# mchitten/keto

Measured on AMD Instinct MI355X. Metric: permission checks/sec (batched, whole node) + traversal HBM GB/s vs roofline, higher is better.
Workload: dtype u32 ids / u64 bitmasks (integer)

## Files before the change

include/ketogpu.h:

```cpp
#ifndef KETOGPU_H
#define KETOGPU_H

#include <stddef.h>
#include <stdint.h>

#ifdef __cplusplus
extern "C" {
#endif

#define KETOGPU_ABI_VERSION 9

#define KETOGPU_OK 0
#define KETOGPU_ENOTFOUND 1
#define KETOGPU_EINVAL 2
#define KETOGPU_EDEVICE 3
#define KETOGPU_ENOMEM 4
#define KETOGPU_ECOLLISION 5

#define KETOGPU_SUBJECT_ID 0
#define KETOGPU_SUBJECT_SET 1
#define KETOGPU_SUBJECT_NIL (-1)

#define KETOGPU_NODE_NONE 0xFFFFFFFFu
#define KETOGPU_NODE_NOT_OWNED 0xFFFFFFFEu
// ... 187 lines not shown
                      uint64_t *allowed_bits, uint64_t *flagged_bits);

size_t ketogpu_packed24_bytes(size_t n);
int ketogpu_pack24(const uint32_t *roots, const uint32_t *targets, size_t n, void *out);
int ketogpu_unpack24(const void *packed, size_t n, uint32_t *roots, uint32_t *targets);
int ketogpu_snapshot_packed24_ok(const ketogpu_snapshot *s);
int ketogpu_check_ids_packed24(ketogpu_engine *e, const void *packed, size_t n, uint64_t *allowed_bits,
                               uint64_t *flagged_bits);
int ketogpu_engine_last_request_path(const ketogpu_engine *e, int32_t *path);

int ketogpu_host_alloc(size_t bytes, void **out);
void ketogpu_host_free(void *p);

typedef struct ketogpu_multi ketogpu_multi;
int ketogpu_multi_new(const ketogpu_snapshot *s, const int32_t *devices, size_t num_devices,
                      const ketogpu_engine_opts *opts, ketogpu_multi **out);
void ketogpu_multi_free(ketogpu_multi *m);
size_t ketogpu_multi_size(const ketogpu_multi *m);
ketogpu_engine *ketogpu_multi_engine(ketogpu_multi *m, size_t i);
int ketogpu_multi_check_ids(ketogpu_multi *m, const uint32_t *roots, const uint32_t *targets, size_t n,
                            uint64_t *allowed_bits, uint64_t *flagged_bits);
int ketogpu_multi_check_ids_packed24(ketogpu_multi *m, const void *packed, size_t n, uint64_t *allowed_bits,
                                     uint64_t *flagged_bits);
void ketogpu_multi_range(size_t n, size_t parts, size_t i, size_t *begin, size_t *end);

int ketogpu_queries_upload(ketogpu_engine *e, const uint32_t *roots, const uint32_t *targets,
                           size_t n, ketogpu_queries **out);
int ketogpu_queries_run(ketogpu_engine *e, ketogpu_queries *q);
int ketogpu_queries_download(ketogpu_engine *e, const ketogpu_queries *q, uint64_t *allowed_bits,
                             uint64_t *flagged_bits);
int ketogpu_queries_run_async(ketogpu_engine *e, ketogpu_queries *q, int *queued);
int ketogpu_engine_wait(ketogpu_engine *e);
int ketogpu_engine_piped_full_requests(ketogpu_engine *e, uint64_t *out);
void ketogpu_queries_free(ketogpu_queries *q);

typedef struct {
    uint64_t checks;
    uint64_t rounds;
    uint64_t levels;
    uint64_t frontier_entries;
    uint64_t interior_edges;
    uint64_t rev_edges;
    uint64_t touched;
    uint64_t bytes_push;
    uint64_t bytes_pull;
    uint64_t bytes_total;
    double ms_push;
    double ms_pull;
    double ms_total;
    uint64_t push_launches;
    uint64_t overflow_retries;
    uint64_t spilled_units;
    uint64_t unit_rows;
    uint64_t unit_edges;
    uint64_t unit_rev;
    uint64_t bytes_unit;
    double ms_unit;
    uint64_t spilled_requests;
    uint64_t unit_launches;
    uint64_t main_bytes;
    double main_ms;
    int32_t plan;
    uint32_t plan_lists;
    uint32_t hubs;
    uint32_t hub_words;
    double hub_build_ms;
// ... 502 lines not shown
    uint32_t slots;
    double last_call_ms;
} ketogpu_expand_stats;
int ketogpu_subjects_expand_stats_get(const ketogpu_subjects *h, ketogpu_expand_stats *out);
int ketogpu_subjects_expand(ketogpu_subjects *h, const uint32_t *roots, const uint32_t *rest_depth, size_t n,
                            uint32_t *out_nodes, uint32_t *out_children, uint64_t capacity, uint64_t *begin,
                            uint64_t *count, uint32_t *status, uint64_t *needed);

typedef struct {
    uint64_t requests;
    uint64_t tier1_requests;
    uint64_t wide_requests;
    uint64_t wide_rounds;
    uint64_t levels;
    uint64_t items;
    uint64_t ids_produced;
    uint64_t truncated_lists;
    uint32_t slots;
    uint32_t chunk;
    double last_call_ms;
} ketogpu_wide_stats;
int ketogpu_subjects_wide_stats_get(const ketogpu_subjects *h, ketogpu_wide_stats *out);
int ketogpu_lookup_wide_stats_get(const ketogpu_lookup *l, ketogpu_wide_stats *out);
int ketogpu_subjects_ids_wide(ketogpu_subjects *h, const uint32_t *roots, size_t n, uint32_t cls, uint32_t *out,
                              uint64_t capacity, uint64_t *begin, uint64_t *count, uint64_t *needed);
int ketogpu_lookup_ids_wide(ketogpu_lookup *l, const uint32_t *targets, size_t n, uint32_t type, uint32_t *out,
                            uint64_t capacity, uint64_t *begin, uint64_t *count, uint64_t *needed);

const char *ketogpu_last_error(void);
int ketogpu_abi_version(void);
void ketogpu_free(void *p);
int ketogpu_device_count(void);
int ketogpu_probe_random_lines(int device, uint64_t table_bytes, uint64_t requests, int reps, double *ms_per_launch);

#ifdef __cplusplus
}
#endif
#endif
```

keto_amd/_lib.py:

```python
import ctypes as C
import os

HERE = os.path.dirname(os.path.abspath(__file__))
LIB_PATH = os.environ.get("KETOGPU_LIB") or os.path.join(HERE, "libketogpu.so")

OK, ENOTFOUND, EINVAL, EDEVICE, ENOMEM, ECOLLISION = 0, 1, 2, 3, 4, 5
SUBJECT_ID, SUBJECT_SET, SUBJECT_NIL = 0, 1, -1
NODE_NONE = 0xFFFFFFFF
NODE_NOT_OWNED = 0xFFFFFFFE
BUILD_SORT = 1
ORDER_NULLS_LAST = 2
ORDERS = {"sqlite": 0, "mysql-bin": 0, "cockroach": 0, "postgres": ORDER_NULLS_LAST}
BUILD_WRITABLE = 4
WRITE_REASONS = {0: "applied", 1: "not_writable", 2: "wildcard", 3: "poison", 4: "class", 5: "ambiguous",
                 6: "full", 7: "reserve", 8: "fanout"}
NODE_UNION, NODE_LEAF = 0, 1
TYPE_ANY, TYPE_NONE = 0xFFFFFFFF, 0xFFFFFFFE
LOOKUP_TRUNCATED, LOOKUP_INVALID = 0xFFFFFFFFFFFFFFFF, 0xFFFFFFFFFFFFFFFE
CLASS_SUBJECT_ID, CLASS_UNTYPED_SET = 0xFFFFFFFD, 0xFFFFFFFC
PAGE_LIMIT_MAX, PAGE_INVALID = 65536, 0xFFFFFFFF
COMBINE_AND, COMBINE_ANDNOT, COMBINE_OR = 0, 1, 2


class KetoError(Exception):
# ... 387 lines not shown
    "ketogpu_core_index_free": (None, [vp]),
    "ketogpu_comm_stats_get": (C.c_int, [vp, C.POINTER(CommStats)]),
    "ketogpu_label_index_build": (C.c_int, [vp, u32, u32, C.POINTER(vp)]),
    "ketogpu_label_index_view": (C.c_int, [vp, C.POINTER(LabelView)]),
    "ketogpu_label_index_free": (None, [vp]),
    "ketogpu_engine_label_heads": (C.c_int, [vp, C.c_int, vp, C.c_uint64, C.POINTER(C.c_uint64),
                                             C.POINTER(C.c_uint32)]),
    "ketogpu_snapshot_save": (C.c_int, [vp, C.c_char_p]),
    "ketogpu_snapshot_apply": (C.c_int, [vp, C.POINTER(RowBatch), C.POINTER(RowBatch), C.POINTER(vp)]),
    "ketogpu_snapshot_load": (C.c_int, [C.c_char_p, C.POINTER(vp)]),
    "ketogpu_snapshot_set_namespaces": (C.c_int, [vp, C.POINTER(Namespace), sz, C.POINTER(vp)]),
    "ketogpu_snapshot_write": (C.c_int, [vp, C.POINTER(RowBatch), C.POINTER(RowBatch), C.POINTER(WriteResult)]),
    "ketogpu_snapshot_version": (C.c_uint64, [vp]),
    "ketogpu_engine_sync": (C.c_int, [vp, C.POINTER(C.c_double), C.POINTER(C.c_uint64)]),
    "ketogpu_engine_check_graph": (C.c_int, [vp, C.POINTER(C.c_uint64)]),
    "ketogpu_resolve": (C.c_int, [vp, C.POINTER(CheckRequest), C.POINTER(u32), C.POINTER(u32)]),
    "ketogpu_resolve_batch": (C.c_int, [vp, C.POINTER(RequestBatch), vp, vp, vp]),
    "ketogpu_engine_new": (C.c_int, [vp, C.POINTER(EngineOpts), C.POINTER(vp)]),
    "ketogpu_engine_free": (None, [vp]),
    "ketogpu_engine_set_events": (C.c_int, [vp, C.c_int]),
    "ketogpu_check": (C.c_int, [vp, C.POINTER(CheckRequest), sz, vp, vp]),
    "ketogpu_check_ids": (C.c_int, [vp, vp, vp, sz, vp, vp]),
    "ketogpu_packed24_bytes": (sz, [sz]),
    "ketogpu_pack24": (C.c_int, [vp, vp, sz, vp]),
    "ketogpu_unpack24": (C.c_int, [vp, sz, vp, vp]),
    "ketogpu_snapshot_packed24_ok": (C.c_int, [vp]),
    "ketogpu_check_ids_packed24": (C.c_int, [vp, vp, sz, vp, vp]),
    "ketogpu_engine_last_request_path": (C.c_int, [vp, C.POINTER(i32)]),
    "ketogpu_queries_upload": (C.c_int, [vp, vp, vp, sz, C.POINTER(vp)]),
    "ketogpu_queries_run": (C.c_int, [vp, vp]),
    "ketogpu_queries_run_async": (C.c_int, [vp, vp, C.POINTER(C.c_int)]),
    "ketogpu_engine_wait": (C.c_int, [vp]),
    "ketogpu_engine_piped_full_requests": (C.c_int, [vp, C.POINTER(C.c_uint64)]),
    "ketogpu_probe_random_lines": (C.c_int, [C.c_int, C.c_uint64, C.c_uint64, C.c_int, C.POINTER(C.c_double)]),
    "ketogpu_queries_download": (C.c_int, [vp, vp, vp, vp]),
    "ketogpu_queries_free": (None, [vp]),
    "ketogpu_engine_last_stats": (C.c_int, [vp, C.POINTER(RunStats)]),
    "ketogpu_expand": (C.c_int, [vp, C.POINTER(Subject), i32, C.POINTER(vp)]),
    "ketogpu_tree_nodes": (C.c_int, [vp, C.POINTER(C.POINTER(TreeNode)), C.POINTER(sz)]),
    "ketogpu_tree_json": (C.c_int, [vp, C.POINTER(vp)]),
    "ketogpu_tree_free": (None, [vp]),
    "ketogpu_last_error": (C.c_char_p, []),
    "ketogpu_abi_version": (C.c_int, []),
    "ketogpu_free": (None, [vp]),
    "ketogpu_device_count": (C.c_int, []),
    "ketogpu_host_alloc": (C.c_int, [sz, C.POINTER(vp)]),
    "ketogpu_host_free": (None, [vp]),
    "ketogpu_multi_new": (C.c_int, [vp, vp, sz, C.POINTER(EngineOpts), C.POINTER(vp)]),
    "ketogpu_multi_free": (None, [vp]),
    "ketogpu_multi_size": (sz, [vp]),
    "ketogpu_multi_engine": (vp, [vp, sz]),
    "ketogpu_multi_check_ids": (C.c_int, [vp, vp, vp, sz, vp, vp]),
    "ketogpu_multi_check_ids_packed24": (C.c_int, [vp, vp, sz, vp, vp]),
    "ketogpu_multi_range": (None, [sz, sz, sz, C.POINTER(sz), C.POINTER(sz)]),
    "ketogpu_shard_builder_new": (C.c_int, [C.POINTER(Namespace), sz, C.POINTER(ShardOpts), C.POINTER(vp)]),
    "ketogpu_shard_builder_append": (C.c_int, [vp, C.POINTER(RowBatch)]),
    "ketogpu_shard_builder_finish": (C.c_int, [vp, C.POINTER(vp)]),
    "ketogpu_shard_builder_free": (None, [vp]),
    "ketogpu_shard_free": (None, [vp]),
    "ketogpu_shard_counts": (C.c_int, [vp, vp]),
    "ketogpu_shard_set_layout": (C.c_int, [vp, vp]),
    "ketogpu_shard_query_count": (C.c_uint64, [vp]),
    "ketogpu_shard_queries": (C.c_int, [vp, vp, C.c_uint64, vp]),
    "ketogpu_shard_answer": (C.c_int, [vp, vp, C.c_uint64, vp]),
    "ketogpu_shard_apply": (C.c_int, [vp, vp, C.c_uint64]),
    "ketogpu_shard_claim_count": (C.c_uint64, [vp]),
    "ketogpu_shard_claims": (C.c_int, [vp, vp, C.c_uint64, vp]),
# ... 132 lines not shown
```

keto_amd/check.py:

```python
import ctypes as C

import numpy as np

from . import _lib as L
from .relationtuple import InternalRelationTuple, NilSubject
from .snapshot import Snapshot, subject_struct


class Engine:
    def __init__(self, snapshot: Snapshot, device=0, max_words_per_round=0, state_budget_bytes=0):
        self.L = L.lib()
        self.snapshot = snapshot
        opts = L.EngineOpts(device, max_words_per_round, state_budget_bytes)
        h = C.c_void_p()
        L.check(self.L.ketogpu_engine_new(snapshot.h, C.byref(opts), C.byref(h)))
        self.h = h
        self.owned = True

    @classmethod
    def borrowed(cls, handle, snapshot, owner):
        e = cls.__new__(cls)
        e.L, e.snapshot, e.h, e.owned, e._owner = L.lib(), snapshot, C.c_void_p(handle), False, owner
        return e

# ... 79 lines not shown
        bad = C.c_uint64()
        L.check(self.L.ketogpu_engine_check_graph(self.h, C.byref(bad)))
        self.check_graph_first = self.L.ketogpu_last_error().decode("utf-8", "replace") if bad.value else ""
        return bad.value

    def label_heads(self, side):
        words, hw = C.c_uint64(), C.c_uint32()
        L.check(self.L.ketogpu_engine_label_heads(self.h, side, None, 0, C.byref(words), C.byref(hw)))
        if not words.value:
            return None, 0
        out = np.empty(words.value, dtype=np.uint32)
        L.check(self.L.ketogpu_engine_label_heads(self.h, side, out.ctypes.data, words.value, C.byref(words),
                                                  C.byref(hw)))
        return out, hw.value

    def sync(self):
        ms, rows = C.c_double(), C.c_uint64()
        L.check(self.L.ketogpu_engine_sync(self.h, C.byref(ms), C.byref(rows)))
        return ms.value, rows.value

    def last_stats(self):
        st = L.RunStats()
        L.check(self.L.ketogpu_engine_last_stats(self.h, C.byref(st)))
        return st.as_dict()

    def wait(self):
        L.check(self.L.ketogpu_engine_wait(self.h))

    def piped_full_requests(self):
        n = C.c_uint64()
        L.check(self.L.ketogpu_engine_piped_full_requests(self.h, C.byref(n)))
        return n.value

    def set_events(self, every_kernel):
        L.check(self.L.ketogpu_engine_set_events(self.h, 1 if every_kernel else 0))


class PinnedBuffer:

    def __init__(self, n, dtype=np.uint32):
        self.L = L.lib()
        dt = np.dtype(dtype)
        p = C.c_void_p()
        L.check(self.L.ketogpu_host_alloc(max(n, 1) * dt.itemsize, C.byref(p)))
        self.p = p
        buf = (C.c_char * (max(n, 1) * dt.itemsize)).from_address(p.value)
        self.array = np.frombuffer(buf, dtype=dt)[:n]

    def close(self):
        if getattr(self, "p", None):
            self.array = None
            self.L.ketogpu_host_free(self.p)
            self.p = None

    def __del__(self):
        self.close()


def pinned(values, dtype=np.uint32):
    values = np.asarray(values, dtype=dtype)
    b = PinnedBuffer(len(values), dtype)
    b.array[:] = values
    return b


class MultiEngine:
# ... 143 lines not shown
```

keto_amd/csrc/device_engine.hip:

```cpp
#include <hip/hip_runtime.h>

#include <algorithm>
#include <atomic>
#include <chrono>
#include <cstring>
#include <functional>
#include <map>
#include <mutex>
#include <string>
#include <thread>
#include <type_traits>
#include <vector>

#include "core_index.hpp"
#include "device_util.hpp"
#include "labels.hpp"
#include "tier.hpp"
#include "ketogpu_internal.hpp"

using namespace ketogpu;
using namespace kdev;

namespace {

// ... 2219 lines not shown
template <int E>
__device__ __forceinline__ bool label_find_e(const uint32_t *L, uint32_t x) {
    const uint32_t pos = label_lower_e<E>(L, x);
    return pos < (uint32_t)E && L[pos] == x;
}

template <int E>
__device__ __forceinline__ bool label_block8(const uint32_t *L, uint32_t x) {
    static_assert(E % 8 == 4, "a head's inline entries");
    constexpr int NB = (E + 7) / 8;
    uint32_t blk = 0;
#pragma unroll
    for (int b = 0; b + 1 < NB; b++) blk += L[8 * b + 7] < x;
    const uint4 u = *reinterpret_cast<const uint4 *>(L + 8 * blk);
    const bool lo = min(min(u.x ^ x, u.y ^ x), min(u.z ^ x, u.w ^ x)) == 0;
    if constexpr (NB == 1) {
        return lo;
    } else {
        const uint4 v = *reinterpret_cast<const uint4 *>(L + 8 * blk + 4);
        const bool hi = min(min(v.x ^ x, v.y ^ x), min(v.z ^ x, v.w ^ x)) == 0;
        return lo | (hi & (blk != (uint32_t)(NB - 1)));
    }
}

template <int E, int H>
__device__ __forceinline__ bool label_lookup(const uint32_t *row, uint32_t x) {
    return label_block8<E>(row + kHeadFixed, x);
}

#ifndef KETO_LABEL_MEET
#define KETO_LABEL_MEET 0
#endif

template <int HS, int HP, bool TAIL = false>
__device__ __forceinline__ void label_unit(LabelShared<HS, HP> &sh, const LabelGraph &L, uint32_t r_lane,
                                           uint32_t t_lane, uint64_t *allowed, const uint64_t unit,
                                           const LabelRest &R, const LabelRest &F, unsigned long long *stats) {
    static_assert((HS == 8 || HS == 16 || HS == 32 || HS == 64) && (HP == 8 || HP == 16 || HP == 32 || HP == 64),
                  "heads of 8, 16, 32 or 64 words");
    constexpr int SW = HS / 4, PW = HP / 4;
    constexpr uint32_t CS = HS - kHeadFixed, CP = HP - kHeadFixed;
    const uint32_t lane = threadIdx.x & 63, q = lane >> 2, sub = lane & 3;
    const uint32_t r = (uint32_t)__shfl((int)r_lane, (int)q, 64), t = (uint32_t)__shfl((int)t_lane, (int)q, 64);
    const bool some = r != KETOGPU_NODE_NONE && t != KETOGPU_NODE_NONE;
    const bool valid = some && r < kDynBase;
    uint32_t sw[SW], pw[PW];
#pragma unroll
    for (int k = 0; k < SW; k++) sw[k] = 0xFFFFFFFFu;
#pragma unroll
    for (int k = 0; k < PW; k++) pw[k] = 0xFFFFFFFFu;
    if (valid) {
        label_head_load<SW>(L.S + (uint64_t)t * HS, sub, sw);
        label_head_load<PW>(L.P + (uint64_t)r * HP, sub, pw);
    }
    const uint32_t ns = label_word<SW, 0>(sw), np = label_word<PW, 0>(pw);
    const bool labelled = valid && ns != kNoLabel && np != kNoLabel;
    const uint64_t smask = (uint64_t)label_word<SW, 2>(sw) | (uint64_t)label_word<SW, 3>(sw) << 32;
    const uint64_t pmask = (uint64_t)label_word<PW, 2>(pw) | (uint64_t)label_word<PW, 3>(pw) << 32;
    uint32_t *Sl = sh.S + q * (HS + 4), *Pl = sh.P + q * (HP + 4);
    label_to_lds<SW>(Sl, sw, sub);
    label_to_lds<PW>(Pl, pw, sub);
    const uint32_t *Se = Sl + kHeadFixed, *Pe = Pl + kHeadFixed;
    const uint32_t shard = (uint32_t)(unit % kRestShards);
    {
        const bool rest = sub == 0 && some && !labelled;
        const uint32_t at = lds_append(rest, R.count + shard * kRestStride);
        if (rest) R.list[shard * R.cap + at] = (uint32_t)(unit * 16 + q);
    }
    wave_sync();
    bool hit = labelled && (smask & pmask) != 0;
    const bool s_body = sub * SW >= kHeadFixed;
    uint32_t es = 0;
#pragma unroll
    for (int k = 0; k < SW; k++) es += (k >= (int)kHeadFixed || s_body) && sw[k] < L.ni;
    es += (uint32_t)__builtin_amdgcn_update_dpp(0, (int)es, 0xB1, 0xf, 0xf, false);
    es += (uint32_t)__builtin_amdgcn_update_dpp(0, (int)es, 0x4E, 0xf, 0xf, false);
    if (!labelled) es = 0;
    const uint32_t ep = min(np, CP);
    {
        bool head = false, body = false;
#pragma unroll
        for (int k = 0; k < SW; k++) (k < (int)kHeadFixed ? head : body) |= sw[k] == r;
        hit |= labelled && r >= L.ni && (body | (head & s_body));
    }
    if (labelled && !hit) {
        if (KETO_LABEL_MEET == 2) {
            if (es <= ep)
// ... 66 lines not shown
            const bool lm_done = es == 0 || np == 0 || (s_whole && (p_whole || s_last <= p_last)) ||
                                 (p_whole && p_last <= s_last);
            const bool raw_done = r < L.ni || ns <= CS || r <= s_end;
            full = !(lm_done && raw_done);
        }
        const uint32_t at = lds_append(full, F.count + shard * kRestStride);
        if (full) {
            uint4 *rec = F.rec + 2 * (shard * F.cap + at);
            rec[0] = make_uint4((uint32_t)(unit * 16 + q), r, t, ns);
            rec[1] = make_uint4(np, os, op, 0u);
        }
    }
    const uint64_t bits = __ballot(hit);
    uint32_t rows = 0, ent = 0;
    if (stats) {
        rows = wave_sum_all(labelled && sub == 0 ? 2u : 0u);
        ent = wave_sum_all(labelled && sub == 0 ? ns + np + kHeadFixed : 0u);
    }
    uint64_t x = bits | bits >> 1;
    x = (x | x >> 2) & 0x1111111111111111ull;
    x = (x | x >> 3) & 0x0303030303030303ull;
    x = (x | x >> 6) & 0x000F000F000F000Full;
    x = (x | x >> 12) & 0x000000FF000000FFull;
    x = (x | x >> 24) & 0xFFFFull;
    if (lane == 0) {
        reinterpret_cast<uint16_t *>(allowed)[unit] = (uint16_t)x;
        if (stats) {
            atomicAdd(&stat_slot(stats)[0], (unsigned long long)rows);
            atomicAdd(&stat_slot(stats)[2], (unsigned long long)ent);
        }
    }
}

__device__ __forceinline__ void label_clear_next(const LabelRest &R, const LabelRest &F) {
    if (blockIdx.x == 0 && threadIdx.x < 64) {
        R.next_count[threadIdx.x * kRestStride] = 0u;
        F.next_count[threadIdx.x * kRestStride] = 0u;
    }
}

template <int HS, int HP>
__global__ __launch_bounds__(64) void label_kernel(LabelGraph L, const uint32_t *roots, const uint32_t *targets,
                                                   uint64_t n, uint64_t *allowed, LabelRest R, LabelRest F,
                                                   unsigned long long *stats, uint64_t unit0) {
    __shared__ LabelShared<HS, HP> sh;
    if (unit0 == 0) label_clear_next(R, F);
    const uint64_t units = (n + 15) / 16;
    const uint64_t unit = unit0 + blockIdx.x;
    uint32_t r, t;
    bidi_load_rt<16>(unit, units, roots, targets, n, r, t);
    label_unit<HS, HP>(sh, L, r, t, allowed, unit, R, F, stats);
    if (unit + 1 == units && threadIdx.x == 0)
        for (uint64_t u = units; u < (units + 3) / 4 * 4; u++) reinterpret_cast<uint16_t *>(allowed)[u] = 0;
}

template <int HS, int HP>
__global__ __launch_bounds__(256) void label_host_kernel(DevGraph g, LabelGraph L, const uint32_t *hr,
                                                         const uint32_t *ht, uint32_t *dr, uint32_t *dt, uint64_t n,
                                                         uint64_t *allowed, LabelRest R, LabelRest F,
                                                         unsigned long long *stats, unsigned long long *first_bad) {
    __shared__ LabelShared<HS, HP> sh[4];
    __shared__ uint32_t rq[2][64];
    const uint32_t wave = threadIdx.x >> 6, lane = threadIdx.x & 63;
    label_clear_next(R, F);
    if (wave == 0) {
        uint32_t r[4], t[4];
        host_unit_requests<4>(g, hr, ht, dr, dt, n, first_bad, r, t);
        if (lane < 16)
#pragma unroll
            for (int k = 0; k < 4; k++) rq[0][16 * k + lane] = r[k], rq[1][16 * k + lane] = t[k];
    }
    __syncthreads();
    const uint64_t units = (n + 15) / 16;
    const uint64_t unit = (uint64_t)blockIdx.x * 4 + wave;
    if (unit >= units) return;
    const uint32_t rk = lane < 16 ? rq[0][16 * wave + lane] : KETOGPU_NODE_NONE;
    const uint32_t tk = lane < 16 ? rq[1][16 * wave + lane] : KETOGPU_NODE_NONE;
    label_unit<HS, HP>(sh[wave], L, rk, tk, allowed, unit, R, F, stats);
}

__device__ __forceinline__ void packed24_decode(uint32_t *raw, const uint64_t *src, uint64_t w0, uint64_t nwords,
                                                uint32_t lane, uint32_t &r, uint32_t &t) {
    if (lane < 48) {
        const uint64_t w = w0 + lane < nwords ? src[w0 + lane] : 0ull;
// ... 115 lines not shown
            for (uint32_t k = sub + 4 * kPre; k < nw && !hit; k += 4) hit = label_find_n(O, nl, W[k]);
            if (sub == 0 && !hit && rr >= L.ni) hit = walk_p ? label_find_n(O, nl, rr) : label_find_n(W, nw, rr);
        }
        const uint64_t bits = __ballot(hit);
        if (valid && sub == 0) {
            if ((bits >> lane) & 0xF) atomicOr((unsigned long long *)&allowed[idx >> 6], 1ull << (idx & 63));
            ent += nl;
        }
        wave_sync();
    }
    return ent;
}

template <int HS, int HP>
__global__ __launch_bounds__(64) void label_full_kernel(LabelGraph L, uint64_t *allowed, LabelRest R, LabelRest F,
                                                        unsigned int *total_rest, unsigned int *total_full,
                                                        unsigned long long *stats, unsigned long long *mirror) {
    constexpr uint32_t kFullStage = full_stage(HS, HP);
    __shared__ alignas(16) uint32_t stage[16 * kFullStage];
    const uint32_t lane = threadIdx.x;
    const uint32_t c = F.count[lane * kRestStride];
    if (blockIdx.x == 0) {
        const uint32_t tr = wave_sum_all(R.count[lane * kRestStride]), tf = wave_sum_all(c);
        if (lane == 0) *total_rest = tr, *total_full = tf;
        if (mirror && lane < 12)
            mirror[lane] = lane == 8 ? (unsigned long long)tr : lane == 11 ? (unsigned long long)tf << 32 : 0ull;
    }
    const uint64_t ent =
        label_dense_units<HS, HP, kFullStage, 16, (int)kFullStage / 16>(stage, L, allowed, F, c, blockIdx.x, gridDim.x);
    const uint32_t e = wave_sum_all((uint32_t)ent);
    if (stats && lane == 0 && e) atomicAdd(&stat_slot(stats)[2], (unsigned long long)e);
}

template <int HS, int HP, bool TAIL>
__global__ __launch_bounds__(64) void label_carry_kernel(LabelGraph L, const uint32_t *roots, const uint32_t *targets,
                                                         uint64_t n, uint64_t *allowed, LabelRest R, LabelRest F,
                                                         LabelRest Fd, uint64_t *allowed_d, uint32_t D) {
    __shared__ LabelShared<HS, HP> sh;
    static_assert(sizeof(LabelShared<HS, HP>) == 64 * (HS + HP + 8), "the dense role's stage");
    if (blockIdx.x < D) {
        label_dense_units<HS, HP, HS + HP + 8, 4, 2>(reinterpret_cast<uint32_t *>(&sh), L, allowed_d, Fd,
                                                     Fd.count[threadIdx.x * kRestStride], blockIdx.x, D);
        return;
    }
    if (blockIdx.x == D) {
        R.next_count[threadIdx.x * kRestStride] = 0u;
        F.next_count[threadIdx.x * kRestStride] = 0u;
    }
    const uint64_t units = (n + 15) / 16;
    const uint64_t unit = blockIdx.x - D;
    uint32_t r, t;
    bidi_load_rt<16>(unit, units, roots, targets, n, r, t);
    label_unit<HS, HP, TAIL>(sh, L, r, t, allowed, unit, R, F, nullptr);
    if (unit + 1 == units && threadIdx.x == 0)
        for (uint64_t u = units; u < (units + 3) / 4 * 4; u++) reinterpret_cast<uint16_t *>(allowed)[u] = 0;
}

template <class SH>
__global__ __launch_bounds__(64) void label_rest_kernel(DevGraph g, const FRec *frec, const FRec *brec,
                                                        const uint32_t *roots, const uint32_t *targets,
                                                        uint64_t *allowed, LabelRest R, unsigned int *total,
                                                        uint32_t *out, unsigned int *out_count,
                                                        unsigned long long *stats) {
    __shared__ SH S;
    const uint32_t lane = threadIdx.x;
    const uint32_t c = R.count[lane * kRestStride];
    const uint32_t nu = (c + 15) / 16;
    const uint32_t incl = wave_incl_sum_u32(nu);
    const uint64_t units = (uint64_t)__builtin_amdgcn_readlane((int)incl, 63);
    const uint32_t listed = wave_sum_all(c);
    if (blockIdx.x == 0 && lane == 0) *total = listed;
    for (uint64_t u = blockIdx.x; u < units; u += gridDim.x) {
        const uint32_t shard = (uint32_t)__builtin_ctzll(__ballot(incl > u));
        const uint32_t first = (uint32_t)__builtin_amdgcn_readlane((int)(incl - nu), (int)shard);
        const uint32_t cs = (uint32_t)__builtin_amdgcn_readlane((int)c, (int)shard);
        const uint64_t j = (u - first) * 16 + lane;
        uint32_t idx = KETOGPU_NODE_NONE, r = KETOGPU_NODE_NONE, t = KETOGPU_NODE_NONE;
        if (lane < 16 && j < cs) {
            idx = R.list[shard * R.cap + j];
            r = roots[idx];
            t = targets[idx];
        }
        lite_unit<SH, false>(S, g, frec, brec, bidi_load_rows(g, r, t), allowed, u, out, out_count, stats, nullptr,
                             idx, true);
        __syncthreads();
    }
// ... 1437 lines not shown
    }();
    bool label_clean = false;
    bool lean_call = false;
    bool pipelined_req = false, queued = false;
    hipStream_t pipe_s[kPipe] = {};
    bool pipe_used[kPipe] = {};
    const ketogpu_queries *pipe_q[kPipe] = {};
    bool label_defer = [] {
        const char *e = getenv("KETOGPU_LABEL_DEFER");
        return !e || atoi(e) != 0;
    }();
    int done_mode = [] {
        const char *e = getenv("KETOGPU_LABEL_DONE_EVENT");
        return !e ? 2 : !strcmp(e, "record") ? 0 : !strcmp(e, "nofence") ? 1 : 2;
    }();
    struct PendingDense {
        bool on = false;
        ketogpu_queries *q = nullptr;
        uint64_t *allowed = nullptr;
        LabelRest R{}, F{};
    } pend[kPipe];
    bool carry_call = false;
    unsigned cur_pipe = 0;
    uint64_t pipe_epoch = 1;
    hipEvent_t order_ev = nullptr;
    hipStream_t pstream(unsigned k) const {
        if (k == cur_pipe) return stream;
        return k ? pipe_s[k] : pipe_s[cur_pipe];
    }
    bool label_tail = [] {
        const char *e = getenv("KETOGPU_LABEL_TAIL");
        return !e || atoi(e) != 0;
    }();
    uint64_t piped_full = 0;
    bool piped_full_known = false, flush_unread = false;
    void take_piped_full() {
        piped_full = ((const unsigned int *)(h_ctr + 24))[7];
        piped_full_known = true;
    }
    static unsigned grid_for(uint64_t full) { return (unsigned)std::min<uint64_t>(std::max<uint64_t>(full / 16 + 64, 64), 16384); }
    unsigned dense_grid() const { return grid_for(full_prev); }
    unsigned piped_grid() const { return grid_for(piped_full_known ? piped_full : full_prev); }
    bool flush_dense(unsigned k) {
        PendingDense p = pend[k];
        if (!p.on) return false;
        pend[k] = PendingDense{};
        label_dispatch([&](auto hs, auto hp) {
            KLAUNCH((label_full_kernel<decltype(hs)::value, decltype(hp)::value>), dim3(piped_grid()), dim3(64), 0,
                    pstream(k), lgraph, p.allowed, p.R, p.F, &spill_count[0], &spill_count[7], nullptr, d_hctr + 16);
        });
        flush_unread = true;
        if (p.q) {
            if (p.q->done_ev) HIP_CHECK(hipEventRecord(p.q->done_ev, pstream(k)));
            p.q->pass = 0;
        }
        return true;
    }
    void flush_dense_all() {
        for (unsigned k = 0; k < kPipe; k++) flush_dense(k);
    }
    void drain_pipe() {
        flush_dense_all();
        for (unsigned k = 0; k < kPipe; k++) {
            pipe_q[k] = nullptr;
            if (pipe_used[k]) HIP_CHECK(hipStreamSynchronize(pstream(k)));
            pipe_used[k] = false;
// ... 66 lines not shown
        return x;
    }
    bool frec_needed = false;
    static constexpr uint64_t kTrialMin = 1 << 16;
    static constexpr int kTrialRuns = 2;
    int trials_left = 0;
    struct Candidate {
        bool bidi;
        int hlog, bt, f, lf;
        double ms;
        bool units = true;
        int u = 16;
        int wpe = 1;
        int lite = 0;
    };
    std::vector<Candidate> candidates;
    struct BidiCfg {
        int hlog, bt, f, lf;
        int u = 16;
        int wpe = 1;
        int lite = 0;
        bool operator==(const BidiCfg &o) const {
            return hlog == o.hlog && bt == o.bt && f == o.f && lf == o.lf && u == o.u && wpe == o.wpe &&
                   lite == o.lite;
        }
    };
    BidiCfg bidi_cfg{9, 64, KETO_F1, 7};

    void launch_bidi(const BidiCfg &c, unsigned grid, unsigned pad, const Batch &q, const uint32_t *parents,
                     const unsigned int *in_count, uint32_t *out, unsigned int *out_count, unsigned long long *stats,
                     unsigned long long *stp, uint64_t unit0 = 0, hipStream_t stream = nullptr, bool chunked = false) {
        if (!stream) stream = this->stream;
        if (c.lite == 3) {
            label_dispatch([&](auto hs, auto hp) {
                KLAUNCH((label_kernel<decltype(hs)::value, decltype(hp)::value>), dim3(grid), dim3(64), pad, stream,
                        lgraph, q.roots, q.targets, q.n, q.allowed, label_rest(q.n), label_full(q.n), stats, unit0);
            });
            return;
        }
        if (c.lite == 2) {
#define KETO_CORE_K(SH)                                                                                       \
    KLAUNCH((lite_kernel<SH, true>), dim3(grid), dim3(64), pad, stream, gcore(), core_rec[0], core_rec[1], q.roots, \
            q.targets, q.n, q.allowed, out, out_count, stats, unit0, stp)
            if (core_shape == 1)
                KETO_CORE_K(CoreShapeS);
            else if (core_shape == 2)
                KETO_CORE_K(CoreShapeM);
            else
                KETO_CORE_K(LiteShape);
#undef KETO_CORE_K
            return;
        }
        if (c.lite) {
            if (c.u == 32)
                KLAUNCH((lite_kernel<LiteShape32>), dim3(grid), dim3(64), pad, stream, g, frec, brec, q.roots,
                        q.targets, q.n, q.allowed, out, out_count, stats, unit0, stp);
            else
                KLAUNCH((lite_kernel<LiteShape>), dim3(grid), dim3(64), pad, stream, g, frec, brec, q.roots, q.targets,
                        q.n, q.allowed, out, out_count, stats, unit0, stp);
            return;
        }
        if (chunked && c == BidiCfg{9, 64, KETO_F1, 7, 16, 1}) {
            KLAUNCH((bidi_kernel<16, 9, KETO_F1, 64, 7, 1, 1>), dim3(grid), dim3(64), pad, stream, g, frec, brec, q.roots,
                    q.targets, q.n, q.allowed, parents, in_count, 1u, out, out_count, stats, stp, unit0);
            return;
        }
#define KETO_BIDI_U(U, HL, F, BT, LF, WPE)                                                                        \
    if (c == BidiCfg{HL, BT, F, LF, U, WPE}) {                                                                   \
        KLAUNCH((bidi_kernel<U, HL, F, BT, LF, WPE>), dim3(grid), dim3(BT), pad, stream, g, frec, brec,          \
// ... 1248 lines not shown
            rs.push_launches++;
            if (!left) return 0;
            HIP_CHECK(hipMemsetAsync(spill_count, 0, sizeof(unsigned int), stream));
            a = ev();
            b = ev();
            HIP_CHECK(hipEventRecord(a, stream));
            KLAUNCH(unit_kernel<1>, dim3((unsigned)(left * wave_u)), dim3(kBlock), 0, stream, g, has_kids,
                               q.roots, q.targets, q.n, q.allowed, q.flags, list[0], (uint32_t)wave_u, list[1],
                               spill_count, st.stats, nullptr);
            HIP_CHECK(hipEventRecord(b, stream));
            unit_ev.push_back({a, b});
            left = read_spill_count();
            rs.spilled_units += left;
            rs.push_launches++;
            if (left)
                HIP_CHECK(hipMemcpyAsync(list[0], list[1], left * sizeof(uint32_t), hipMemcpyDeviceToDevice, stream));
            return left;
        }
        uint64_t units = (q.n + 15) / 16;
        uint64_t left = 0;
        if (use_v2 || (use_lite && use_bidi)) {
            if (use_bidi) {
                const bool direct = src && src->mapped && pipe_direct &&
                                    (bidi_cfg == BidiCfg{9, 64, KETO_F1, 7, 16, 1} || bidi_cfg.lite);
                const bool light = light_begin && (direct || !src);
                hipEvent_t a = light ? light_begin : ev(), b = light ? nullptr : ev();
                if (!light) HIP_CHECK(hipEventRecord(a, stream));
                const uint64_t bunits = (q.n + bidi_cfg.u - 1) / bidi_cfg.u;
                if (!src && carry_call) {
                    PendingDense p = pend[cur_pipe];
                    pend[cur_pipe] = PendingDense{};
                    const unsigned D = p.on ? piped_grid() : 0u;
                    label_dispatch([&](auto hs, auto hp) {
                        if (label_tail)
                            KLAUNCH((label_carry_kernel<decltype(hs)::value, decltype(hp)::value, true>),
                                    dim3(D + (unsigned)bunits), dim3(64), lds_pad, stream, lgraph, q.roots, q.targets,
                                    q.n, q.allowed, label_rest(q.n), label_full(q.n), p.F, p.allowed, D);
                        else
                            KLAUNCH((label_carry_kernel<decltype(hs)::value, decltype(hp)::value, false>),
                                    dim3(D + (unsigned)bunits), dim3(64), lds_pad, stream, lgraph, q.roots, q.targets,
                                    q.n, q.allowed, label_rest(q.n), label_full(q.n), p.F, p.allowed, D);
                    });
                    if (p.q) p.q->pass = 2;
                } else if (!src) {
                    launch_bidi(bidi_cfg, (unsigned)bunits, lds_pad, q, nullptr, nullptr, list[0], &spill_count[0],
                                lean_call ? nullptr : st.stats, stamps);
                } else if (direct) {
#define KETO_HOST_K(K)                                                                                     \
    do {                                                                                                   \
        if (bidi_cfg.lite == 3)                                                                            \
            launch_label_host(q, src, bunits);                                                             \
        else if (bidi_cfg.lite == 2 && core_shape == 1)                                                    \
            KLAUNCH((lite_host_kernel<K, CoreShapeS, true>), dim3((unsigned)((bunits + K - 1) / K)), dim3(64), \
                    0, stream, gcore(), core_rec[0], core_rec[1], src->roots, src->targets, io->d_roots,   \
                    io->d_targets, q.n, q.allowed, list[0], &spill_count[0], st.stats, d_bad);              \
        else if (bidi_cfg.lite == 2 && core_shape == 2)                                                    \
            KLAUNCH((lite_host_kernel<K, CoreShapeM, true>), dim3((unsigned)((bunits + K - 1) / K)), dim3(64), \
                    0, stream, gcore(), core_rec[0], core_rec[1], src->roots, src->targets, io->d_roots,   \
                    io->d_targets, q.n, q.allowed, list[0], &spill_count[0], st.stats, d_bad);              \
        else if (bidi_cfg.lite == 2)                                                                       \
            KLAUNCH((lite_host_kernel<K, LiteShape, true>), dim3((unsigned)((bunits + K - 1) / K)), dim3(64), \
                    0, stream, gcore(), core_rec[0], core_rec[1], src->roots, src->targets, io->d_roots,   \
                    io->d_targets, q.n, q.allowed, list[0], &spill_count[0], st.stats, d_bad);              \
        else if (bidi_cfg.lite && bidi_cfg.u == 32)                                                        \
            KLAUNCH((lite_host_kernel<K, LiteShape32>), dim3((unsigned)((bunits + K - 1) / K)), dim3(64), 0, \
                    stream, g, frec, brec, src->roots, src->targets, io->d_roots, io->d_targets, q.n,      \
                    q.allowed, list[0], &spill_count[0], st.stats, d_bad);                                 \
        else if (bidi_cfg.lite)                                                                            \
            KLAUNCH((lite_host_kernel<K, LiteShape>), dim3((unsigned)((bunits + K - 1) / K)), dim3(64), 0,   \
                    stream, g, frec, brec, src->roots, src->targets, io->d_roots, io->d_targets, q.n,      \
                    q.allowed, list[0], &spill_count[0], st.stats, d_bad);                                 \
        else                                                                                               \
            KLAUNCH(bidi_host_kernel<K>, dim3((unsigned)((bunits + K - 1) / K)), dim3(64), 0, stream, g,   \
                    frec, brec, src->roots, src->targets, io->d_roots, io->d_targets, q.n, q.allowed,      \
                    list[0], &spill_count[0], st.stats, d_bad);                                            \
// ... 747 lines not shown
        else if (q->pass == 0)
            q->pass = 2;
        q->last_s = si;
        q->pending = true;
        e->pipe_q[si] = q;
        e->pipe_used[si] = true;
    } else {
        e->pipe_q[si] = nullptr;
        q->pending = false;
    }
    e->pipelined_req = false;
    if (queued) *queued = e->queued ? 1 : 0;
    API_END
}

int ketogpu_engine_wait(ketogpu_engine *e) {
    API_BEGIN
    if (!e) throw Error(KETOGPU_EINVAL, "null argument");
    std::lock_guard<std::mutex> lk(e->mu);
    HIP_CHECK(hipSetDevice(e->device));
    e->drain_pipe();
    HIP_CHECK(hipStreamSynchronize(e->stream));
    API_END
}

int ketogpu_engine_piped_full_requests(ketogpu_engine *e, uint64_t *out) {
    API_BEGIN
    if (!e || !out) throw Error(KETOGPU_EINVAL, "null argument");
    std::lock_guard<std::mutex> lk(e->mu);
    *out = e->piped_full_known ? e->piped_full : 0;
    API_END
}

int ketogpu_queries_download(ketogpu_engine *e, const ketogpu_queries *q, uint64_t *allowed_bits,
                             uint64_t *flagged_bits) {
    API_BEGIN
    if (!e || !q) throw Error(KETOGPU_EINVAL, "null argument");
    std::lock_guard<std::mutex> lk(e->mu);
    e->download(const_cast<ketogpu_queries &>(*q), allowed_bits, flagged_bits);
    API_END
}

void ketogpu_queries_free(ketogpu_queries *q) {
    if (q && q->pass == 1 && q->eng) {
        ketogpu_engine *e = q->eng;
        std::lock_guard<std::mutex> lk(e->mu);
        try {
            HIP_CHECK(hipSetDevice(e->device));
            for (unsigned k = 0; k < ketogpu_engine::kPipe; k++)
                if (e->pend[k].on && e->pend[k].q == q) e->flush_dense(k);
        } catch (const Error &) {
            for (unsigned k = 0; k < ketogpu_engine::kPipe; k++)
                if (e->pend[k].q == q) e->pend[k] = ketogpu_engine::PendingDense{};
        }
    }
    delete q;
}

int ketogpu_check_ids(ketogpu_engine *e, const uint32_t *roots, const uint32_t *targets, size_t n,
                      uint64_t *allowed_bits, uint64_t *flagged_bits) {
    API_BEGIN
    if (!e || (n && (!roots || !targets || !allowed_bits))) throw Error(KETOGPU_EINVAL, "null argument");
    std::shared_lock<std::shared_mutex> rd(e->snap->mu);
    std::lock_guard<std::mutex> lk(e->mu);
    e->sync();
    e->check_host(roots, targets, n, allowed_bits, flagged_bits);
// ... 216 lines not shown
```

keto_amd/csrc/probe.hip:

```cpp
#include <hip/hip_runtime.h>

#include <cstdint>

#include "../../include/ketogpu.h"

namespace {

__global__ __launch_bounds__(64) void probe_lines_kernel(const uint32_t *table, uint64_t lines, const uint32_t *rq,
                                                         uint64_t n, uint16_t *out) {
    const uint32_t lane = threadIdx.x, q = lane >> 2, sub = lane & 3;
    const uint64_t i0 = (uint64_t)blockIdx.x * 16;
    uint32_t a = 0, b = 0;
    if (lane < 16 && i0 + lane < n) a = rq[2 * (i0 + lane)], b = rq[2 * (i0 + lane) + 1];
    a = (uint32_t)__shfl((int)a, (int)q, 64);
    b = (uint32_t)__shfl((int)b, (int)q, 64);
    uint32_t v = 0;
    if (i0 + q < n) {
        const uint4 *x = reinterpret_cast<const uint4 *>(table + (a % lines) * 32) + 2 * sub;
        const uint4 *y = reinterpret_cast<const uint4 *>(table + (b % lines) * 32) + 2 * sub;
        const uint4 x0 = x[0], x1 = x[1], y0 = y[0], y1 = y[1];
        v = x0.x ^ x0.y ^ x0.z ^ x0.w ^ x1.x ^ x1.y ^ x1.z ^ x1.w ^ y0.x ^ y0.y ^ y0.z ^ y0.w ^ y1.x ^ y1.y ^ y1.z ^ y1.w;
    }
    const uint64_t bits = __ballot((v & 0xF) == 3);
    if (lane == 0) out[blockIdx.x] = (uint16_t)(bits ^ (bits >> 16) ^ (bits >> 32) ^ (bits >> 48));
}

}

extern "C" int ketogpu_probe_random_lines(int device, uint64_t table_bytes, uint64_t requests, int reps,
                                          double *ms_per_launch) {
    if (!ms_per_launch || requests == 0 || reps <= 0 || table_bytes < (1u << 20)) return KETOGPU_EINVAL;
    *ms_per_launch = 0;
    if (hipSetDevice(device) != hipSuccess) return KETOGPU_EDEVICE;
    const uint64_t lines = table_bytes / 128;
    uint32_t *table = nullptr, *rq = nullptr;
    uint16_t *out = nullptr;
    hipStream_t s = nullptr;
    hipEvent_t e0 = nullptr, e1 = nullptr;
    int rc = KETOGPU_OK;
    auto ok = [&](hipError_t e) {
        if (e != hipSuccess && rc == KETOGPU_OK) rc = e == hipErrorOutOfMemory ? KETOGPU_ENOMEM : KETOGPU_EDEVICE;
        return rc == KETOGPU_OK;
    };
    const uint64_t grid = (requests + 15) / 16;
    if (ok(hipMalloc(&table, lines * 128)) && ok(hipMalloc(&rq, 8 * requests)) && ok(hipMalloc(&out, 2 * grid)) &&
        ok(hipStreamCreateWithFlags(&s, hipStreamNonBlocking)) && ok(hipEventCreate(&e0)) && ok(hipEventCreate(&e1)) &&
        ok(hipMemsetAsync(table, 0x5a, lines * 128, s))) {
        uint32_t *h = nullptr;
        if (ok(hipHostMalloc(&h, 8 * requests, hipHostMallocDefault))) {
            uint64_t x = 88172645463325252ull;
            for (uint64_t k = 0; k < 2 * requests; k++) {
                x ^= x << 13, x ^= x >> 7, x ^= x << 17;
                h[k] = (uint32_t)(x >> 17);
            }
            if (ok(hipMemcpyAsync(rq, h, 8 * requests, hipMemcpyHostToDevice, s)) && ok(hipStreamSynchronize(s))) {
                for (int k = 0; k < 3 && rc == KETOGPU_OK; k++)
                    probe_lines_kernel<<<dim3((unsigned)grid), dim3(64), 0, s>>>(table, lines, rq, requests, out);
                ok(hipGetLastError());
                if (ok(hipEventRecord(e0, s))) {
                    for (int k = 0; k < reps && rc == KETOGPU_OK; k++)
                        probe_lines_kernel<<<dim3((unsigned)grid), dim3(64), 0, s>>>(table, lines, rq, requests, out);
                    ok(hipGetLastError());
                    float ms = 0;
                    if (ok(hipEventRecord(e1, s)) && ok(hipEventSynchronize(e1)) && ok(hipEventElapsedTime(&ms, e0, e1)))
                        *ms_per_launch = ms / reps;
                }
            }
            (void)hipHostFree(h);
        }
    }
    if (s) (void)hipStreamSynchronize(s);
    if (e0) (void)hipEventDestroy(e0);
    if (e1) (void)hipEventDestroy(e1);
    if (s) (void)hipStreamDestroy(s);
    for (void *p : {(void *)table, (void *)rq, (void *)out})
        if (p) (void)hipFree(p);
    return rc;
}
```

Measured before the change: 24.90 billion.

## Process two label units per wave to overlap head loads in carry kernel

Splits label_unit into a head-load phase and a settle phase, then adds a paired variant that issues the random head loads for two 16-query units before settling either one. The goal is to raise memory-level parallelism on the latency-bound random-line gathers and halve the block count. It is on by default in the carry kernel when both head sizes are 32. The sync path only uses it with KETOGPU_LABEL_PAIR>=2. It costs extra registers for the second unit's heads, which may lower occupancy, and it adds a multi-stream variant of the random-line probe.

```diff
diff --git a/include/ketogpu.h b/include/ketogpu.h
--- a/include/ketogpu.h
+++ b/include/ketogpu.h
@@ -243,6 +243,7 @@
 int ketogpu_queries_run_async(ketogpu_engine *e, ketogpu_queries *q, int *queued);
 int ketogpu_engine_wait(ketogpu_engine *e);
 int ketogpu_engine_piped_full_requests(ketogpu_engine *e, uint64_t *out);
+int ketogpu_engine_label_pair_launches(ketogpu_engine *e, uint64_t *out);
 void ketogpu_queries_free(ketogpu_queries *q);
 
 typedef struct {
@@ -811,6 +812,8 @@
 void ketogpu_free(void *p);
 int ketogpu_device_count(void);
 int ketogpu_probe_random_lines(int device, uint64_t table_bytes, uint64_t requests, int reps, double *ms_per_launch);
+int ketogpu_probe_random_lines_streams(int device, uint64_t table_bytes, uint64_t requests, int reps, int streams,
+                                       double *ms_per_launch);
 
 #ifdef __cplusplus
 }
diff --git a/keto_amd/_lib.py b/keto_amd/_lib.py
--- a/keto_amd/_lib.py
+++ b/keto_amd/_lib.py
@@ -443,7 +443,10 @@
     "ketogpu_queries_run_async": (C.c_int, [vp, vp, C.POINTER(C.c_int)]),
     "ketogpu_engine_wait": (C.c_int, [vp]),
     "ketogpu_engine_piped_full_requests": (C.c_int, [vp, C.POINTER(C.c_uint64)]),
+    "ketogpu_engine_label_pair_launches": (C.c_int, [vp, C.POINTER(C.c_uint64)]),
     "ketogpu_probe_random_lines": (C.c_int, [C.c_int, C.c_uint64, C.c_uint64, C.c_int, C.POINTER(C.c_double)]),
+    "ketogpu_probe_random_lines_streams": (C.c_int, [C.c_int, C.c_uint64, C.c_uint64, C.c_int, C.c_int,
+                                                     C.POINTER(C.c_double)]),
     "ketogpu_queries_download": (C.c_int, [vp, vp, vp, vp]),
     "ketogpu_queries_free": (None, [vp]),
     "ketogpu_engine_last_stats": (C.c_int, [vp, C.POINTER(RunStats)]),
diff --git a/keto_amd/check.py b/keto_amd/check.py
--- a/keto_amd/check.py
+++ b/keto_amd/check.py
@@ -135,6 +135,11 @@
         L.check(self.L.ketogpu_engine_piped_full_requests(self.h, C.byref(n)))
         return n.value
 
+    def label_pair_launches(self):
+        n = C.c_uint64()
+        L.check(self.L.ketogpu_engine_label_pair_launches(self.h, C.byref(n)))
+        return n.value
+
     def set_events(self, every_kernel):
         L.check(self.L.ketogpu_engine_set_events(self.h, 1 if every_kernel else 0))
 
diff --git a/keto_amd/csrc/device_engine.hip b/keto_amd/csrc/device_engine.hip
--- a/keto_amd/csrc/device_engine.hip
+++ b/keto_amd/csrc/device_engine.hip
@@ -2275,19 +2275,13 @@
 #define KETO_LABEL_MEET 0
 #endif
 
-template <int HS, int HP, bool TAIL = false>
-__device__ __forceinline__ void label_unit(LabelShared<HS, HP> &sh, const LabelGraph &L, uint32_t r_lane,
-                                           uint32_t t_lane, uint64_t *allowed, const uint64_t unit,
-                                           const LabelRest &R, const LabelRest &F, unsigned long long *stats) {
-    static_assert((HS == 8 || HS == 16 || HS == 32 || HS == 64) && (HP == 8 || HP == 16 || HP == 32 || HP == 64),
-                  "heads of 8, 16, 32 or 64 words");
+
+template <int HS, int HP>
+__device__ __forceinline__ void label_heads(const LabelGraph &L, uint32_t r, uint32_t t, uint32_t (&sw)[HS / 4],
+                                            uint32_t (&pw)[HP / 4]) {
     constexpr int SW = HS / 4, PW = HP / 4;
-    constexpr uint32_t CS = HS - kHeadFixed, CP = HP - kHeadFixed;
-    const uint32_t lane = threadIdx.x & 63, q = lane >> 2, sub = lane & 3;
-    const uint32_t r = (uint32_t)__shfl((int)r_lane, (int)q, 64), t = (uint32_t)__shfl((int)t_lane, (int)q, 64);
-    const bool some = r != KETOGPU_NODE_NONE && t != KETOGPU_NODE_NONE;
-    const bool valid = some && r < kDynBase;
-    uint32_t sw[SW], pw[PW];
+    const uint32_t sub = threadIdx.x & 3;
+    const bool valid = r != KETOGPU_NODE_NONE && t != KETOGPU_NODE_NONE && r < kDynBase;
 #pragma unroll
     for (int k = 0; k < SW; k++) sw[k] = 0xFFFFFFFFu;
 #pragma unroll
@@ -2296,6 +2290,20 @@
         label_head_load<SW>(L.S + (uint64_t)t * HS, sub, sw);
         label_head_load<PW>(L.P + (uint64_t)r * HP, sub, pw);
     }
+}
+
+template <int HS, int HP, bool TAIL>
+__device__ __forceinline__ void label_settle(LabelShared<HS, HP> &sh, const LabelGraph &L, const uint32_t r,
+                                             const uint32_t t, const uint32_t (&sw)[HS / 4],
+                                             const uint32_t (&pw)[HP / 4], uint64_t *allowed, const uint64_t unit,
+                                             const LabelRest &R, const LabelRest &F, unsigned long long *stats) {
+    static_assert((HS == 8 || HS == 16 || HS == 32 || HS == 64) && (HP == 8 || HP == 16 || HP == 32 || HP == 64),
+                  "heads of 8, 16, 32 or 64 words");
+    constexpr int SW = HS / 4, PW = HP / 4;
+    constexpr uint32_t CS = HS - kHeadFixed, CP = HP - kHeadFixed;
+    const uint32_t lane = threadIdx.x & 63, q = lane >> 2, sub = lane & 3;
+    const bool some = r != KETOGPU_NODE_NONE && t != KETOGPU_NODE_NONE;
+    const bool valid = some && r < kDynBase;
     const uint32_t ns = label_word<SW, 0>(sw), np = label_word<PW, 0>(pw);
     const bool labelled = valid && ns != kNoLabel && np != kNoLabel;
     const uint64_t smask = (uint64_t)label_word<SW, 2>(sw) | (uint64_t)label_word<SW, 3>(sw) << 32;
@@ -2428,6 +2436,42 @@
     }
 }
 
+template <int HS, int HP, bool TAIL = false>
+__device__ __forceinline__ void label_unit(LabelShared<HS, HP> &sh, const LabelGraph &L, uint32_t r_lane,
+                                           uint32_t t_lane, uint64_t *allowed, const uint64_t unit,
+                                           const LabelRest &R, const LabelRest &F, unsigned long long *stats) {
+    const uint32_t q = (threadIdx.x & 63) >> 2;
+    const uint32_t r = (uint32_t)__shfl((int)r_lane, (int)q, 64), t = (uint32_t)__shfl((int)t_lane, (int)q, 64);
+    uint32_t sw[HS / 4], pw[HP / 4];
+    label_heads<HS, HP>(L, r, t, sw, pw);
+    label_settle<HS, HP, TAIL>(sh, L, r, t, sw, pw, allowed, unit, R, F, stats);
+}
+
+template <int HS, int HP, bool TAIL>
+__device__ __forceinline__ void label_pair(LabelShared<HS, HP> &sh, const LabelGraph &L, const uint32_t *roots,
+                                           const uint32_t *targets, uint64_t n, uint64_t *allowed,
+                                           const uint64_t unit, const bool two, const LabelRest &R,
+                                           const LabelRest &F, unsigned long long *stats) {
+    const uint32_t lane = threadIdx.x & 63, q = lane >> 2;
+    const uint64_t c = unit * 16 + (lane & 31);
+    uint32_t v = KETOGPU_NODE_NONE;
+    if (c < n) v = (lane < 32 ? roots : targets)[c];
+    const uint32_t r0 = (uint32_t)__shfl((int)v, (int)q, 64), t0 = (uint32_t)__shfl((int)v, (int)(32 + q), 64);
+    uint32_t r1 = KETOGPU_NODE_NONE, t1 = KETOGPU_NODE_NONE;
+    if (two) {
+        r1 = (uint32_t)__shfl((int)v, (int)(16 + q), 64);
+        t1 = (uint32_t)__shfl((int)v, (int)(48 + q), 64);
+    }
+    uint32_t sw0[HS / 4], pw0[HP / 4], sw1[HS / 4], pw1[HP / 4];
+    label_heads<HS, HP>(L, r0, t0, sw0, pw0);
+    label_heads<HS, HP>(L, r1, t1, sw1, pw1);
+    label_settle<HS, HP, TAIL>(sh, L, r0, t0, sw0, pw0, allowed, unit, R, F, stats);
+    if (two) {
+        wave_sync();
+        label_settle<HS, HP, TAIL>(sh, L, r1, t1, sw1, pw1, allowed, unit + 1, R, F, stats);
+    }
+}
+
 __device__ __forceinline__ void label_clear_next(const LabelRest &R, const LabelRest &F) {
     if (blockIdx.x == 0 && threadIdx.x < 64) {
         R.next_count[threadIdx.x * kRestStride] = 0u;
@@ -2435,17 +2479,25 @@
     }
 }
 
-template <int HS, int HP>
+template <int HS, int HP, bool PAIR = false>
 __global__ __launch_bounds__(64) void label_kernel(LabelGraph L, const uint32_t *roots, const uint32_t *targets,
                                                    uint64_t n, uint64_t *allowed, LabelRest R, LabelRest F,
                                                    unsigned long long *stats, uint64_t unit0) {
     __shared__ LabelShared<HS, HP> sh;
     if (unit0 == 0) label_clear_next(R, F);
     const uint64_t units = (n + 15) / 16;
-    const uint64_t unit = unit0 + blockIdx.x;
-    uint32_t r, t;
-    bidi_load_rt<16>(unit, units, roots, targets, n, r, t);
-    label_unit<HS, HP>(sh, L, r, t, allowed, unit, R, F, stats);
+    uint64_t unit;
+    if constexpr (PAIR) {
+        unit = unit0 + 2 * (uint64_t)blockIdx.x;
+        const bool two = unit + 1 < units;
+        label_pair<HS, HP, false>(sh, L, roots, targets, n, allowed, unit, two, R, F, stats);
+        unit += two;
+    } else {
+        unit = unit0 + blockIdx.x;
+        uint32_t r, t;
+        bidi_load_rt<16>(unit, units, roots, targets, n, r, t);
+        label_unit<HS, HP>(sh, L, r, t, allowed, unit, R, F, stats);
+    }
     if (unit + 1 == units && threadIdx.x == 0)
         for (uint64_t u = units; u < (units + 3) / 4 * 4; u++) reinterpret_cast<uint16_t *>(allowed)[u] = 0;
 }
@@ -2627,7 +2679,7 @@
     if (stats && lane == 0 && e) atomicAdd(&stat_slot(stats)[2], (unsigned long long)e);
 }
 
-template <int HS, int HP, bool TAIL>
+template <int HS, int HP, bool TAIL, bool PAIR = false>
 __global__ __launch_bounds__(64) void label_carry_kernel(LabelGraph L, const uint32_t *roots, const uint32_t *targets,
                                                          uint64_t n, uint64_t *allowed, LabelRest R, LabelRest F,
                                                          LabelRest Fd, uint64_t *allowed_d, uint32_t D) {
@@ -2643,10 +2695,18 @@
         F.next_count[threadIdx.x * kRestStride] = 0u;
     }
     const uint64_t units = (n + 15) / 16;
-    const uint64_t unit = blockIdx.x - D;
-    uint32_t r, t;
-    bidi_load_rt<16>(unit, units, roots, targets, n, r, t);
-    label_unit<HS, HP, TAIL>(sh, L, r, t, allowed, unit, R, F, nullptr);
+    uint64_t unit;
+    if constexpr (PAIR) {
+        unit = 2 * (uint64_t)(blockIdx.x - D);
+        const bool two = unit + 1 < units;
+        label_pair<HS, HP, TAIL>(sh, L, roots, targets, n, allowed, unit, two, R, F, nullptr);
+        unit += two;
+    } else {
+        unit = blockIdx.x - D;
+        uint32_t r, t;
+        bidi_load_rt<16>(unit, units, roots, targets, n, r, t);
+        label_unit<HS, HP, TAIL>(sh, L, r, t, allowed, unit, R, F, nullptr);
+    }
     if (unit + 1 == units && threadIdx.x == 0)
         for (uint64_t u = units; u < (units + 3) / 4 * 4; u++) reinterpret_cast<uint16_t *>(allowed)[u] = 0;
 }
@@ -4150,6 +4210,13 @@
         const char *e = getenv("KETOGPU_LABEL_TAIL");
         return !e || atoi(e) != 0;
     }();
+    int label_pair_mode = [] {
+        const char *e = getenv("KETOGPU_LABEL_PAIR");
+        return e ? atoi(e) : 1;
+    }();
+    bool pair_carry() const { return label_pair_mode >= 2 || (label_pair_mode == 1 && label_hs == 32 && label_hp == 32); }
+    bool pair_sync() const { return label_pair_mode >= 2; }
+    uint64_t pair_launches = 0;
     uint64_t piped_full = 0;
     bool piped_full_known = false, flush_unread = false;
     void take_piped_full() {
@@ -4282,9 +4349,17 @@
                      unsigned long long *stp, uint64_t unit0 = 0, hipStream_t stream = nullptr, bool chunked = false) {
         if (!stream) stream = this->stream;
         if (c.lite == 3) {
+            const bool pair = pair_sync() && unit0 % 2 == 0 && (grid % 2 == 0 || unit0 + grid == (q.n + 15) / 16);
+            pair_launches += pair;
             label_dispatch([&](auto hs, auto hp) {
-                KLAUNCH((label_kernel<decltype(hs)::value, decltype(hp)::value>), dim3(grid), dim3(64), pad, stream,
-                        lgraph, q.roots, q.targets, q.n, q.allowed, label_rest(q.n), label_full(q.n), stats, unit0);
+                if (pair)
+                    KLAUNCH((label_kernel<decltype(hs)::value, decltype(hp)::value, true>), dim3((grid + 1) / 2),
+                            dim3(64), pad, stream, lgraph, q.roots, q.targets, q.n, q.allowed, label_rest(q.n),
+                            label_full(q.n), stats, unit0);
+                else
+                    KLAUNCH((label_kernel<decltype(hs)::value, decltype(hp)::value>), dim3(grid), dim3(64), pad,
+                            stream, lgraph, q.roots, q.targets, q.n, q.allowed, label_rest(q.n), label_full(q.n),
+                            stats, unit0);
             });
             return;
         }
@@ -5599,15 +5674,19 @@
                     pend[cur_pipe] = PendingDense{};
                     const unsigned D = p.on ? piped_grid() : 0u;
                     label_dispatch([&](auto hs, auto hp) {
-                        if (label_tail)
-                            KLAUNCH((label_carry_kernel<decltype(hs)::value, decltype(hp)::value, true>),
-                                    dim3(D + (unsigned)bunits), dim3(64), lds_pad, stream, lgraph, q.roots, q.targets,
-                                    q.n, q.allowed, label_rest(q.n), label_full(q.n), p.F, p.allowed, D);
-                        else
-                            KLAUNCH((label_carry_kernel<decltype(hs)::value, decltype(hp)::value, false>),
-                                    dim3(D + (unsigned)bunits), dim3(64), lds_pad, stream, lgraph, q.roots, q.targets,
-                                    q.n, q.allowed, label_rest(q.n), label_full(q.n), p.F, p.allowed, D);
+                        auto go = [&](auto tail, auto pair) {
+                            const unsigned first = (unsigned)(decltype(pair)::value ? (bunits + 1) / 2 : bunits);
+                            KLAUNCH((label_carry_kernel<decltype(hs)::value, decltype(hp)::value,
+                                                        decltype(tail)::value, decltype(pair)::value>),
+                                    dim3(D + first), dim3(64), lds_pad, stream, lgraph, q.roots, q.targets, q.n,
+                                    q.allowed, label_rest(q.n), label_full(q.n), p.F, p.allowed, D);
+                        };
+                        if (label_tail && pair_carry()) go(std::true_type{}, std::true_type{});
+                        else if (label_tail) go(std::true_type{}, std::false_type{});
+                        else if (pair_carry()) go(std::false_type{}, std::true_type{});
+                        else go(std::false_type{}, std::false_type{});
                     });
+                    pair_launches += pair_carry();
                     if (p.q) p.q->pass = 2;
                 } else if (!src) {
                     launch_bidi(bidi_cfg, (unsigned)bunits, lds_pad, q, nullptr, nullptr, list[0], &spill_count[0],
@@ -6421,6 +6500,14 @@
     API_END
 }
 
+int ketogpu_engine_label_pair_launches(ketogpu_engine *e, uint64_t *out) {
+    API_BEGIN
+    if (!e || !out) throw Error(KETOGPU_EINVAL, "null argument");
+    std::lock_guard<std::mutex> lk(e->mu);
+    *out = e->pair_launches;
+    API_END
+}
+
 int ketogpu_queries_download(ketogpu_engine *e, const ketogpu_queries *q, uint64_t *allowed_bits,
                              uint64_t *flagged_bits) {
     API_BEGIN
diff --git a/keto_amd/csrc/probe.hip b/keto_amd/csrc/probe.hip
--- a/keto_amd/csrc/probe.hip
+++ b/keto_amd/csrc/probe.hip
@@ -27,25 +27,31 @@
 
 }
 
-extern "C" int ketogpu_probe_random_lines(int device, uint64_t table_bytes, uint64_t requests, int reps,
-                                          double *ms_per_launch) {
-    if (!ms_per_launch || requests == 0 || reps <= 0 || table_bytes < (1u << 20)) return KETOGPU_EINVAL;
+extern "C" int ketogpu_probe_random_lines_streams(int device, uint64_t table_bytes, uint64_t requests, int reps,
+                                                  int streams, double *ms_per_launch) {
+    constexpr int kMaxStreams = 8;
+    if (!ms_per_launch || requests == 0 || reps <= 0 || table_bytes < (1u << 20) || streams < 1 ||
+        streams > kMaxStreams)
+        return KETOGPU_EINVAL;
     *ms_per_launch = 0;
     if (hipSetDevice(device) != hipSuccess) return KETOGPU_EDEVICE;
     const uint64_t lines = table_bytes / 128;
     uint32_t *table = nullptr, *rq = nullptr;
     uint16_t *out = nullptr;
-    hipStream_t s = nullptr;
-    hipEvent_t e0 = nullptr, e1 = nullptr;
+    hipStream_t s[kMaxStreams] = {};
+    hipEvent_t e0 = nullptr, e1 = nullptr, end[kMaxStreams] = {};
     int rc = KETOGPU_OK;
     auto ok = [&](hipError_t e) {
         if (e != hipSuccess && rc == KETOGPU_OK) rc = e == hipErrorOutOfMemory ? KETOGPU_ENOMEM : KETOGPU_EDEVICE;
         return rc == KETOGPU_OK;
     };
     const uint64_t grid = (requests + 15) / 16;
-    if (ok(hipMalloc(&table, lines * 128)) && ok(hipMalloc(&rq, 8 * requests)) && ok(hipMalloc(&out, 2 * grid)) &&
-        ok(hipStreamCreateWithFlags(&s, hipStreamNonBlocking)) && ok(hipEventCreate(&e0)) && ok(hipEventCreate(&e1)) &&
-        ok(hipMemsetAsync(table, 0x5a, lines * 128, s))) {
+    for (int k = 0; k < streams && rc == KETOGPU_OK; k++)
+        if (ok(hipStreamCreateWithFlags(&s[k], hipStreamNonBlocking)))
+            ok(hipEventCreateWithFlags(&end[k], hipEventDisableTiming));
+    if (rc == KETOGPU_OK && ok(hipMalloc(&table, lines * 128)) && ok(hipMalloc(&rq, 8 * requests)) &&
+        ok(hipMalloc(&out, 2 * grid * streams)) && ok(hipEventCreate(&e0)) && ok(hipEventCreate(&e1)) &&
+        ok(hipMemsetAsync(table, 0x5a, lines * 128, s[0]))) {
         uint32_t *h = nullptr;
         if (ok(hipHostMalloc(&h, 8 * requests, hipHostMallocDefault))) {
             uint64_t x = 88172645463325252ull;
@@ -53,27 +59,42 @@
                 x ^= x << 13, x ^= x >> 7, x ^= x << 17;
                 h[k] = (uint32_t)(x >> 17);
             }
-            if (ok(hipMemcpyAsync(rq, h, 8 * requests, hipMemcpyHostToDevice, s)) && ok(hipStreamSynchronize(s))) {
-                for (int k = 0; k < 3 && rc == KETOGPU_OK; k++)
-                    probe_lines_kernel<<<dim3((unsigned)grid), dim3(64), 0, s>>>(table, lines, rq, requests, out);
+            auto launch = [&](int k) {
+                probe_lines_kernel<<<dim3((unsigned)grid), dim3(64), 0, s[k % streams]>>>(table, lines, rq, requests,
+                                                                                          out + grid * (k % streams));
+            };
+            if (ok(hipMemcpyAsync(rq, h, 8 * requests, hipMemcpyHostToDevice, s[0])) && ok(hipStreamSynchronize(s[0]))) {
+                for (int k = 0; k < 3 * streams && rc == KETOGPU_OK; k++) launch(k);
                 ok(hipGetLastError());
-                if (ok(hipEventRecord(e0, s))) {
-                    for (int k = 0; k < reps && rc == KETOGPU_OK; k++)
-                        probe_lines_kernel<<<dim3((unsigned)grid), dim3(64), 0, s>>>(table, lines, rq, requests, out);
+                for (int k = 1; k < streams; k++) ok(hipStreamSynchronize(s[k]));
+                if (ok(hipEventRecord(e0, s[0]))) {
+                    for (int k = 1; k < streams; k++) ok(hipStreamWaitEvent(s[k], e0, 0));
+                    for (int k = 0; k < reps && rc == KETOGPU_OK; k++) launch(k);
                     ok(hipGetLastError());
+                    for (int k = 1; k < streams; k++)
+                        if (ok(hipEventRecord(end[k], s[k]))) ok(hipStreamWaitEvent(s[0], end[k], 0));
                     float ms = 0;
-                    if (ok(hipEventRecord(e1, s)) && ok(hipEventSynchronize(e1)) && ok(hipEventElapsedTime(&ms, e0, e1)))
+                    if (ok(hipEventRecord(e1, s[0])) && ok(hipEventSynchronize(e1)) && ok(hipEventElapsedTime(&ms, e0, e1)))
                         *ms_per_launch = ms / reps;
                 }
             }
             (void)hipHostFree(h);
         }
     }
-    if (s) (void)hipStreamSynchronize(s);
-    if (e0) (void)hipEventDestroy(e0);
-    if (e1) (void)hipEventDestroy(e1);
-    if (s) (void)hipStreamDestroy(s);
+    for (int k = 0; k < streams; k++)
+        if (s[k]) (void)hipStreamSynchronize(s[k]);
+    for (hipEvent_t e : {e0, e1})
+        if (e) (void)hipEventDestroy(e);
+    for (int k = 0; k < streams; k++) {
+        if (end[k]) (void)hipEventDestroy(end[k]);
+        if (s[k]) (void)hipStreamDestroy(s[k]);
+    }
     for (void *p : {(void *)table, (void *)rq, (void *)out})
         if (p) (void)hipFree(p);
     return rc;
 }
+
+extern "C" int ketogpu_probe_random_lines(int device, uint64_t table_bytes, uint64_t requests, int reps,
+                                          double *ms_per_launch) {
+    return ketogpu_probe_random_lines_streams(device, table_bytes, requests, reps, 1, ms_per_launch);
+}
```

Result: faster. 25.79 billion (median of 6 runs) (+3.6%).
